# Pixel-Talk/CanonSwap

Hardware: AMD Instinct MI355X
Metric: frames/sec at 512x512 (generator hot path F->W->T->R->W->G) (higher is better)
Workload: dtype f16; 1 GPU; BASELINE configs[2]: 512x512 video, 64 frames batched per launch on each GPU, steady state over 1280 frames (20 launches per GPU) (256x256 crops in, random-init weights of the real architecture); frames_per_launch_per_gpu=64, frames_total=1280, parallelism=frame-shard x1, identities_resident=1, latency_mode=False, accumulate=fp32, debug_decodes=False

## Files before the change

canonswap_amd/csrc/vol32.hip:

```cpp
#include "conv_epilogue.h"

namespace {

constexpr int V_TW = 8;
constexpr int V_NC = V_TW + 2;
constexpr int V_CS = 17 * 16;
constexpr int V_RS = V_NC * V_CS;
constexpr int V_WLO = 27 * 2 * 1024;
constexpr int V_SROWS = 8;
enum { V_EPI_F16 = 0,
       V_EPI_RES = 1,
       V_EPI_STAT = 2 };

template <bool SPLIT, int EPI = 0> struct VRing {
    static constexpr int K = SPLIT ? 2 : 4;
    static constexpr int RING = K + 2;
    static constexpr int QS = ((RING * V_RS + 16 + 255) / 256) * 256;
    static constexpr int IMG = 4 * QS;
    static constexpr int NIMG = SPLIT ? 2 : 1;
    static constexpr int AUX = NIMG * IMG;
    static constexpr int RROWS = K + 1;
    static constexpr int RSLOT = 4 * 4096;
    static constexpr int lds(int epi) { return AUX + (SPLIT ? V_WLO : 0) + (epi == 1 ? RROWS * RSLOT : 0); }
};

struct Vol32Params {
    const half_t* in; const half_t* zero;
    int in_sN, in_sH, in_sW;
    int N, H, W;
    const half_t* wgt;
    const float* bias;
    float sl0, sl1;
    const float* res; int res_sN, res_sH, res_sW;
    void* out0; int o0_sN, o0_sH, o0_sW;
    half_t* out1; int o1_sN, o1_sH, o1_sW;
    const float* s2; const float* t2;
    float* stat_out; int stat_nblk;
    int srows;
    const float* xf_y; int xy_sN, xy_sH, xy_sW;
    const float* xf_res; int xr_sN, xr_sH, xr_sW;
    float* xf_out; int xo_sN, xo_sH, xo_sW;
    const float* xf_stats; const float* xf_gamma; const float* xf_beta; float xf_slope;
    int nstrips, nseg, seg_rows, items;
#ifdef V32_TL
    unsigned long long* tl; long tl_cap;
#endif
};

typedef unsigned int u4v __attribute__((ext_vector_type(4)));

#ifdef V32_TL
#define TLS(i) do { __builtin_amdgcn_sched_barrier(0); const unsigned long long t_ = __builtin_amdgcn_s_memtime(); tl_acc[i] += t_ - tl_last; tl_last = t_; \
                    __builtin_amdgcn_sched_barrier(0); } while (0)
#else
#define TLS(i) do { } while (0)
#endif

template <int N> __device__ __forceinline__ void wait_vm() { asm volatile("s_waitcnt vmcnt(%0)" ::"n"(N) : "memory"); }

template <int EPI, bool SPLIT, int XF>
__global__ void __launch_bounds__(256, 1) vol32_kernel(const Vol32Params p)
{
    static_assert(XF == 0 || (SPLIT && EPI == V_EPI_STAT), "transform staging exists for the split-precision statistics kernel");
    extern __shared__ __attribute__((aligned(16))) unsigned char smem[];
    using R = VRing<SPLIT, EPI>;
    constexpr int K = R::K, RING = R::RING, QS = R::QS, IMG = R::IMG, NIMG = R::NIMG;
    constexpr int VOX = SPLIT ? 64 : 32;
    static_assert(!(SPLIT && EPI == V_EPI_RES), "the residual ring and the W_lo fragments share the LDS region after the images");
    constexpr int ND = XF ? 0 : 3 * NIMG + (EPI == V_EPI_RES ? 4 : 0), NR = 0, NS = EPI == V_EPI_F16 ? 2 : (EPI == V_EPI_RES ? 6 : 4);
    constexpr int NW0 = NR + (K - 2) * (ND + NR + NS), NW = NW0 + NS;
    static_assert(NW <= 63, "vmcnt is a 6-bit counter");
    const int tid = threadIdx.x, lane = tid & 63;
    const int wave = __builtin_amdgcn_readfirstlane(tid >> 6);
    const int l15 = lane & 15, l4 = lane >> 4;
#ifdef V32_TL
    unsigned long long tl_acc[10] = {0, 0, 0, 0, 0, 0, 0, 0, 0, 0}, tl_last = __builtin_amdgcn_s_memtime();
#endif

    for (int i = tid * 16; i < NIMG * IMG; i += 256 * 16) *(u4v*)(smem + i) = (u4v){0u, 0u, 0u, 0u};
    h8_t wr[27][2];
    {
        const half_t* wl = p.wgt + ep_lane_row(1, l15) * 32 + l4 * 8;
#pragma unroll
        for (int t = 0; t < 27; ++t) {
            wr[t][0] = *(const h8_t*)(wl + t * 1024 + ep_frag_row(1, 0) * 32);
            wr[t][1] = *(const h8_t*)(wl + t * 1024 + ep_frag_row(1, 1) * 32);
        }
        if constexpr (SPLIT) {
            for (int f = wave; f < 54; f += 4) {
                const h8_t v = *(const h8_t*)(wl + (27 + (f >> 1)) * 1024 + ep_frag_row(1, f & 1) * 32);
                *(h8_t*)(smem + R::AUX + f * 1024 + lane * 16) = v;
            }
        }
    }
    float bias_v[8], s2_v[8], t2_v[8];
#pragma unroll
    for (int r = 0; r < 8; ++r) {
        bias_v[r] = p.bias ? p.bias[l4 * 8 + r] : 0.f;
        s2_v[r] = p.s2 ? p.s2[l4 * 8 + r] : 1.f;
        t2_v[r] = p.s2 ? p.t2[l4 * 8 + r] : 0.f;
    }
    __syncthreads();

    int s_off[3]; bool s_on[3];
#pragma unroll
    for (int j = 0; j < 3; ++j) {
        const int idx = j * 64 + lane, col = idx / 17, ds = idx % 17;
        s_on[j] = idx < V_NC * 17 && ds != 0;
        s_off[j] = col * p.in_sW + (ds - 1) * VOX + wave * 8;
    }
    const int lanebase = l4 * QS + l15 * 16 + (2 * wave) * V_CS;
    const unsigned lane_el = (unsigned)(l15 * 32 + l4 * 8);
    const unsigned char* wlo = smem + R::AUX + lane * 16;

    const int G = (int)gridDim.x;
    int u = (int)blockIdx.x;
    if ((G & 7) == 0) u = (u & 7) * (G >> 3) + (u >> 3);

    for (int item = u; item < p.items; item += G) {
        int t = item;
        const int strip = t % p.nstrips; t /= p.nstrips;
        const int seg = t % p.nseg;
        const int n = t / p.nseg;
        const int w0 = strip * V_TW;
        const int h0 = seg * p.seg_rows, h1 = (h0 + p.seg_rows < p.H) ? h0 + p.seg_rows : p.H;
        bool c_ok[3];
#pragma unroll
        for (int j = 0; j < 3; ++j) {
            const int col = (j * 64 + lane) / 17;
            c_ok[j] = s_on[j] && (unsigned)(w0 - 1 + col) < (unsigned)p.W;
        }
        const half_t* in_n = p.in + (long)n * p.in_sN + (long)(w0 - 1) * p.in_sW;
        const unsigned nb_o0 = (unsigned)(n * p.o0_sN + (w0 + 2 * wave) * p.o0_sW);
        const unsigned nb_o1 = (unsigned)(n * p.o1_sN + (w0 + 2 * wave) * p.o1_sW);
        const unsigned nb_rs = (unsigned)(n * p.res_sN + (w0 + 2 * wave) * p.res_sW);
        auto stage_piece = [&](int r, int slot, int rslot, int q) {
            if (q < 3 * NIMG) {
                const int im = q / 3, j = q % 3;
                const bool rok = (unsigned)r < (unsigned)p.H && r <= h1;
                const half_t* rp = in_n + (long)r * p.in_sH;
                unsigned char* dst = smem + wave * QS + slot * V_RS;
                if (s_on[j]) {
                    const half_t* src = (rok && c_ok[j]) ? rp + s_off[j] + im * 32 : p.zero;
                    __builtin_amdgcn_global_load_lds((const __attribute__((address_space(1))) void*)src,
                                                     (__attribute__((address_space(3))) void*)(dst + im * IMG + j * 1024), 16, 0, 0);
                }
            } else if constexpr (EPI == V_EPI_RES) {
                const int j = q - 3 * NIMG;
                const int rc = (unsigned)r < (unsigned)p.H ? r : 0;
                const float* rsrc = p.res + (nb_rs + (unsigned)(rc * p.res_sH) + lane_el);
                unsigned char* rdst = smem + R::AUX + rslot * R::RSLOT + wave * 4096;
                __builtin_amdgcn_global_load_lds((const __attribute__((address_space(1))) void*)(rsrc + (j >> 1) * p.res_sW + (j & 1) * 4),
                                                 (__attribute__((address_space(3))) void*)(rdst + j * 1024), 16, 0, 0);
            }
        };
        auto stage_row = [&](int r, int slot, int rslot) {
#pragma unroll
            for (int q = 0; q < ND; ++q) stage_piece(r, slot, rslot, q);
        };
        constexpr bool XRES = XF >= 2 && ((XF - 2) & 1) != 0, XWB = XF >= 2 && ((XF - 2) & 2) != 0;
        float4 xr[XF ? 3 : 1][2], xs[XRES ? 3 : 1][2];
        float xsc[XF >= 2 ? 8 : 1], xsh[XF >= 2 ? 8 : 1];
        const int xq = tid & 3;
        if constexpr (XF >= 2) {
#pragma unroll
            for (int r = 0; r < 8; ++r) {
                const int c = xq * 8 + r;
                const float mean = p.xf_stats[((long)n * 32 + c) * 2], rstd = p.xf_stats[((long)n * 32 + c) * 2 + 1];
                xsc[r] = gn_scale(rstd, p.xf_gamma[c]);
                xsh[r] = gn_shift(mean, xsc[r], p.xf_beta[c]);
            }
        }
        int xoff[XF ? 3 : 1]; bool xcok[XF ? 3 : 1];
        if constexpr (XF != 0) {
#pragma unroll
            for (int it = 0; it < 3; ++it) {
                int idx = it * 256 + tid;
                if (idx >= V_NC * 64) idx -= 128;
                const int col = idx >> 6, d = (idx >> 2) & 15;
                xoff[it] = n * p.xy_sN + (w0 - 1 + col) * p.xy_sW + d * 32 + xq * 8;
                xcok[it] = (unsigned)(w0 - 1 + col) < (unsigned)p.W;
            }
        }
        const unsigned xsafe = (unsigned)(n * p.xy_sN + w0 * p.xy_sW + h0 * p.xy_sH + ((tid >> 2) & 15) * 32 + xq * 8);
        auto xf_load_to = [&](int r, int it, float4 (&dr)[2], float4 (&ds)[2]) {
            if constexpr (XF != 0) {
                const bool okl = xcok[it] && (unsigned)r < (unsigned)p.H && r <= h1;
                const unsigned o = okl ? (unsigned)(xoff[it] + r * p.xy_sH) : xsafe;
                const float* y = p.xf_y + o;
                dr[0] = *(const float4*)y; dr[1] = *(const float4*)(y + 4);
                if constexpr (XRES) {
                    const float* x = p.xf_res + o;
                    ds[0] = *(const float4*)x; ds[1] = *(const float4*)(x + 4);
                }
            }
        };
        auto xf_load = [&](int r, int it) { xf_load_to(r, it, xr[it], xs[XRES ? it : 0]); };
        float xa[8];
        auto xf_write_from = [&](int r, int slot, int it, int part, const float4 (&xr)[2], const float4 (&xs)[2]) {
            if constexpr (XF != 0) {
                int idx = it * 256 + tid;
                if (idx >= V_NC * 64) idx -= 128;
                const bool ok = xcok[it] && (unsigned)r < (unsigned)p.H && r <= h1;
#pragma unroll
                for (int k = 0; k < 8; ++k) {
                    if (part >= 0 && (k >> 2) != part) continue;
                    const float v = ((const float*)&xr[k >> 2])[k & 3];
                    if constexpr (XRES) xa[k] = gn_lrelu(v, xsc[k], xsh[k], ((const float*)&xs[k >> 2])[k & 3], p.xf_slope);
                    else if constexpr (XF >= 2) xa[k] = gn_lrelu(v, xsc[k], xsh[k], 0.f, p.xf_slope);
                    else xa[k] = v;
                    if (!ok) xa[k] = 0.f;
                }
                if (part >= 0 && part != 2) return;
                h8_t hi, lo;
#pragma unroll
                for (int k = 0; k < 8; ++k) { hi[k] = (half_t)xa[k]; lo[k] = (half_t)(xa[k] - (float)hi[k]); }
                unsigned char* dst = smem + xq * QS + (idx >> 6) * V_CS + (((idx >> 2) & 15) + 1) * 16 + slot * V_RS;
                *(h8_t*)dst = hi; *(h8_t*)(dst + IMG) = lo;
                if constexpr (XWB) {
                    float* o = ok ? p.xf_out + (unsigned)(xoff[it] + r * p.xy_sH) : (float*)p.zero;
                    *(float4*)o = make_float4(xa[0], xa[1], xa[2], xa[3]); *(float4*)(o + 4) = make_float4(xa[4], xa[5], xa[6], xa[7]);
                }
            }
        };
        auto xf_write = [&](int r, int slot, int it, int part) { xf_write_from(r, slot, it, part, xr[it], xs[XRES ? it : 0]); };
        if constexpr (XF != 0) {
            float4 pr[3][3][2], ps[XRES ? 3 : 1][3][2];
#pragma unroll
            for (int i = 0; i < 3; ++i)
#pragma unroll
                for (int it = 0; it < 3; ++it) xf_load_to(h0 - 1 + i, it, pr[i][it], ps[XRES ? i : 0][it]);
#pragma unroll
            for (int i = 0; i < 3; ++i)
#pragma unroll
                for (int it = 0; it < 3; ++it) xf_write_from(h0 - 1 + i, i, it, -1, pr[i][it], ps[XRES ? i : 0][it]);
        } else {
#pragma unroll
            for (int i = 0; i <= K; ++i) stage_row(h0 - 1 + i, i, i == 0 ? K : i - 1);
        }
        TLS(0);
        __syncthreads();
        TLS(1);

        float ov[2][8]; h8_t ou[2];
        bool have = false;
        int hprev = 0;
        auto store_piece = [&](int k) {
            constexpr int PC = NS / 2;
            const int c = k / PC, w = k % PC;
            const unsigned o = nb_o0 + (unsigned)(hprev * p.o0_sH + c * p.o0_sW) + lane_el;
            if constexpr (EPI != V_EPI_F16) {
                if (w == 0) *(float4*)((float*)p.out0 + o) = make_float4(ov[c][0], ov[c][1], ov[c][2], ov[c][3]);
                if (w == 1) *(float4*)((float*)p.out0 + o + 4) = make_float4(ov[c][4], ov[c][5], ov[c][6], ov[c][7]);
                if constexpr (EPI == V_EPI_RES) {
                    if (w == 2) *(h8_t*)(p.out1 + (nb_o1 + (unsigned)(hprev * p.o1_sH + c * p.o1_sW) + lane_el)) = ou[c];
                }
            } else {
                h8_t x;
#pragma unroll
                for (int r = 0; r < 8; ++r) x[r] = ep_h(ov[c][r]);
                *(h8_t*)((half_t*)p.out0 + o) = x;
            }
        };
        auto flush = [&]() {
#pragma unroll
            for (int k = 0; k < NS; ++k) store_piece(k);
        };
        float st_s[8], st_q[8];
#pragma unroll
        for (int r = 0; r < 8; ++r) { st_s[r] = 0.f; st_q[r] = 0.f; }

        int s0 = 0, r0 = 0;
        for (int h = h0; h < h1; ++h) {
            int sk = s0 + K + 1; sk -= sk >= RING ? RING : 0;
            int rk = r0 + K; rk -= rk >= R::RROWS ? R::RROWS : 0;
            f4_t rr[2][2];
            if constexpr (EPI == V_EPI_RES) {
#pragma unroll
                for (int c = 0; c < 2; ++c)
#pragma unroll
                    for (int i = 0; i < 2; ++i) rr[c][i] = *(const f4_t*)(wlo + r0 * R::RSLOT + wave * 4096 + (c * 2 + i) * 1024);
            }
            int rb[3];
#pragma unroll
            for (int kh = 0; kh < 3; ++kh) { int sl = s0 + kh; sl -= sl >= RING ? RING : 0; rb[kh] = lanebase + sl * V_RS; }
            f4_t acc[2][2];
#pragma unroll
            for (int c = 0; c < 2; ++c)
#pragma unroll
                for (int ci = 0; ci < 2; ++ci) acc[c][ci] = (f4_t){0.f, 0.f, 0.f, 0.f};
            constexpr int NG = SPLIT ? 27 : 9;
            constexpr int XL0 = 4, XW0 = 17;
            h8_t fa[4], fb[4];
            h8_t wa[SPLIT ? 3 : 1][2], wb[SPLIT ? 3 : 1][2];
            auto rd = [&](h8_t (&f)[4], h8_t (&wl2)[SPLIT ? 3 : 1][2], int G2) {
                const int pass = G2 / 9, g = G2 % 9, kd = g / 3, kh = g % 3;
                const int img = (SPLIT && pass == 2) ? IMG : 0;
#pragma unroll
                for (int i = 0; i < 4; ++i) f[i] = *(const h8_t*)(smem + rb[kh] + img + i * V_CS + kd * 16);
                if constexpr (SPLIT) {
                    if (pass == 1) {
#pragma unroll
                        for (int kw = 0; kw < 3; ++kw)
#pragma unroll
                            for (int ci = 0; ci < 2; ++ci) wl2[kw][ci] = *(const h8_t*)(wlo + ((g * 3 + kw) * 2 + ci) * 1024);
                    }
                }
            };
            rd(fa, wa, 0);
#pragma unroll
            for (int G2 = 0; G2 < NG; ++G2) {
                h8_t (&cur)[4] = (G2 & 1) ? fb : fa;
                h8_t (&wcur)[SPLIT ? 3 : 1][2] = (G2 & 1) ? wb : wa;
                h8_t (&wnxt)[SPLIT ? 3 : 1][2] = (G2 & 1) ? wa : wb;
                if constexpr (XF != 0) { if (G2 >= XW0 && G2 < XW0 + 9) xf_write(h + 2, sk, (G2 - XW0) / 3, (G2 - XW0) % 3); }
                if (G2 + 1 < NG) {
                    h8_t (&nxt)[4] = (G2 & 1) ? fa : fb;
                    rd(nxt, wnxt, G2 + 1);
                }
                const int pass = G2 / 9, g = G2 % 9;
#pragma unroll
                for (int kw = 0; kw < 3; ++kw)
#pragma unroll
                    for (int c = 0; c < 2; ++c)
#pragma unroll
                        for (int ci = 0; ci < 2; ++ci) {
                            const h8_t a = (SPLIT && pass == 1) ? wcur[SPLIT ? kw : 0][ci] : wr[g * 3 + kw][ci];
                            acc[c][ci] = __builtin_amdgcn_mfma_f32_16x16x32_f16(a, cur[kw + c], acc[c][ci], 0, 0, 0);
                        }
                if (G2 + 1 < NG) {
                    const int nrd = 4 + ((SPLIT && (G2 + 1) / 9 == 1) ? 6 : 0);
                    const bool conv_here = XF != 0 && G2 >= XW0 && G2 < XW0 + 9;
#pragma unroll
                    for (int i = 0; i < 11; ++i) {
                        __builtin_amdgcn_sched_group_barrier(0x008, 1, 0);
                        if (i < nrd) __builtin_amdgcn_sched_group_barrier(0x100, 1, 0);
                        if (conv_here) __builtin_amdgcn_sched_group_barrier(0x002, 4, 0);
                    }
                }
                __builtin_amdgcn_sched_barrier(0);
                if constexpr (XF == 0) {
                    constexpr int NM = ND + NS;
#pragma unroll
                    for (int m = G2 * NM / NG; m < (G2 + 1) * NM / NG; ++m) {
                        asm volatile("" ::: "memory");
                        if (m < ND) stage_piece(h + K, sk, rk, m);
                        else if (have) store_piece(m - ND);
                        asm volatile("" ::: "memory");
                    }
                    __builtin_amdgcn_sched_barrier(0);
                } else {
                    if (G2 < NS && have) store_piece(G2);
                    if (G2 >= XL0 && G2 < XL0 + 6 && ((G2 - XL0) & 1) == 0) xf_load(h + 2, (G2 - XL0) >> 1);
                    __builtin_amdgcn_sched_barrier(0);
                }
            }
            TLS(4);
#pragma unroll
            for (int c = 0; c < 2; ++c) {
#pragma unroll
                for (int r = 0; r < 8; ++r) {
                    float v = acc[c][r >> 2][r & 3] + bias_v[r];
                    v = lin_act(v, p.sl0);
                    if constexpr (EPI == V_EPI_RES) v += rr[c][r >> 2][r & 3];
                    ov[c][r] = v;
                    if constexpr (EPI == V_EPI_STAT) { st_s[r] += v; st_q[r] = fmaf(v, v, st_q[r]); }
                    if constexpr (EPI == V_EPI_RES) {
                        const float a = v * s2_v[r] + t2_v[r];
                        ou[c][r] = ep_h(lin_act(a, p.sl1));
                    }
                }
            }
            if constexpr (EPI == V_EPI_STAT) {
                if (((h + 1) % p.srows) == 0 || h + 1 == h1) {
                    const int blk = (h / p.srows) * (p.W / 2) + (w0 / 2 + wave);
                    float pa[8], pb[8];
#pragma unroll
                    for (int r = 0; r < 8; ++r) {
                        float a = st_s[r], b = st_q[r];
                        st_s[r] = 0.f; st_q[r] = 0.f;
#pragma unroll
                        for (int o = 1; o < 16; o <<= 1) { a += __shfl_xor(a, o, 64); b += __shfl_xor(b, o, 64); }
                        pa[r] = a; pb[r] = b;
                    }
                    if (l15 == 0) {
                        float4* dst = (float4*)(p.stat_out + (((long)n * p.stat_nblk + blk) * 32 + l4 * 8) * 2);
#pragma unroll
                        for (int r = 0; r < 4; ++r) dst[r] = make_float4(pa[2 * r], pb[2 * r], pa[2 * r + 1], pb[2 * r + 1]);
                    }
                }
            }
            have = true; hprev = h;
            s0 = s0 + 1 == RING ? 0 : s0 + 1;
            r0 = r0 + 1 == R::RROWS ? 0 : r0 + 1;
            TLS(5);
            if constexpr (XF != 0) asm volatile("s_waitcnt lgkmcnt(0)" ::: "memory");
            else if (h > h0 + K - 2) wait_vm<NW>();
            else wait_vm<NW0>();
            TLS(6);
            __builtin_amdgcn_s_barrier();
            asm volatile("" ::: "memory");
            TLS(7);
#ifdef V32_TL
            tl_acc[9] += 1;
#endif
        }
        if (have) flush();
        __syncthreads();
        TLS(8);
    }
#ifdef V32_TL
    if (p.tl && lane == 0) {
        const long wi = (long)blockIdx.x * 4 + wave;
        if (wi < p.tl_cap) {
            unsigned hwid;
            asm volatile("s_getreg_b32 %0, hwreg(HW_REG_HW_ID)" : "=s"(hwid));
            unsigned long long* o = p.tl + wi * 12;
#pragma unroll
            for (int i = 0; i < 10; ++i) o[i] = tl_acc[i];
            o[10] = hwid; o[11] = __builtin_amdgcn_s_memrealtime();
        }
    }
#endif
}

int g_ncu = 0;
#ifdef V32_TL
unsigned long long* g_v32_tl = nullptr;
long g_v32_cap = 0;
#endif

}

#ifdef V32_TL
extern "C" void cs_debug_set_vol32_tl(void* buf, long cap) { g_v32_tl = (unsigned long long*)buf; g_v32_cap = cap; }
#endif

bool vol32_supported(const ConvParams& p)
{
    if (p.KD != 3 || p.KH != 3 || p.KW != 3 || p.Cout_pad != 32 || p.Cout != 32 || p.D != 16 || p.inD != 16 || (p.W % V_TW) != 0) return false;
    if (p.xf_kind) {
        if (!p.hilo || p.Cin != 96 || !p.stat_out || (p.xf_kind != 1 && p.xf_kind != 2) || !p.xf_y.p || p.xf_y.sD != 32) return false;
        if (p.xf_kind == 2 && (!p.xf_stats || !p.xf_gamma || !p.xf_beta)) return false;
        if (p.xf_res.p && (p.xf_kind != 2 || p.xf_res.sD != 32)) return false;
        if (p.xf_out.p && (p.xf_kind != 2 || p.xf_out.sD != 32)) return false;
    } else if (p.hilo ? (p.Cin != 96 || p.in_sD != 64) : (p.Cin != 32 || p.in_sD != 32)) return false;
    if (p.up_shift || p.cg || p.wslot || p.sk_out || p.ragged || p.pixscale || p.stats || p.pool_hw || p.spmul) return false;
    if (p.act0 > ACT_LRELU || p.act1 > ACT_LRELU) return false;
    if (p.res.p && (!p.res_f32 || p.res.sD != 32)) return false;
    if (p.out0.p && p.out0.sD != 32) return false;
    if (p.out1.p && p.out1.sD != 32) return false;
    if (!p.out0.p) return false;
    if (p.hilo && !p.stat_out) return false;
    if (p.stat_out) return p.out0_f32 && !p.res.p && !p.out1.p;
    if (p.res.p) return p.out0_f32 && p.out1.p && !p.hilo;
    return !p.out0_f32 && !p.out1.p;
}

static int vol32_srows(const ConvParams& p) { return p.v32_srows > 0 ? p.v32_srows : V_SROWS; }
int vol32_stat_nblk(const ConvParams& p) { const int sr = vol32_srows(p); return ((p.H + sr - 1) / sr) * (p.W / 2); }

int launch_vol32(const ConvParams& p, hipStream_t st)
{
    if (!vol32_supported(p)) { cs_set_error("vol32: not a 3x3x3 32 -> 32 convolution on a [N][H][W][16][32] volume this kernel supports"); return -1; }
    if (ep_check_extents(p, "vol32")) return -1;
    const long in_span = (long)(p.N - 1) * p.in_sN + (long)(p.H - 1) * p.in_sH + (long)(p.W - 1) * p.in_sW + 1024;
    if (!p.xf_kind && in_span >= (1L << 31)) { cs_set_error("vol32: the input spans 2^31 elements or more"); return -1; }
    if (!g_ncu) {
        int dev = 0, n = 0;
        if (hipGetDevice(&dev) != hipSuccess || hipDeviceGetAttribute(&n, hipDeviceAttributeMultiprocessorCount, dev) != hipSuccess || n < 1) n = 256;
        g_ncu = n;
    }
    Vol32Params k;
    k.in = p.in; k.zero = p.zero; k.in_sN = (int)p.in_sN; k.in_sH = (int)p.in_sH; k.in_sW = (int)p.in_sW;
    k.N = p.N; k.H = p.H; k.W = p.W;
    k.wgt = p.wgt; k.bias = p.bias;
    k.sl0 = p.act0 == ACT_NONE ? 1.f : (p.act0 == ACT_LRELU ? p.slope0 : 0.f);
    k.sl1 = p.act1 == ACT_NONE ? 1.f : (p.act1 == ACT_LRELU ? p.slope1 : 0.f);
    k.res = (const float*)p.res.p; k.res_sN = (int)p.res.sN; k.res_sH = (int)p.res.sH; k.res_sW = (int)p.res.sW;
    k.out0 = p.out0.p; k.o0_sN = (int)p.out0.sN; k.o0_sH = (int)p.out0.sH; k.o0_sW = (int)p.out0.sW;
    k.out1 = (half_t*)p.out1.p; k.o1_sN = (int)p.out1.sN; k.o1_sH = (int)p.out1.sH; k.o1_sW = (int)p.out1.sW;
    k.s2 = p.s2; k.t2 = p.t2;
    k.stat_out = p.stat_out; k.stat_nblk = vol32_stat_nblk(p); k.srows = vol32_srows(p);
    k.xf_y = (const float*)p.xf_y.p; k.xy_sN = (int)p.xf_y.sN; k.xy_sH = (int)p.xf_y.sH; k.xy_sW = (int)p.xf_y.sW;
    k.xf_res = (const float*)p.xf_res.p; k.xr_sN = (int)p.xf_res.sN; k.xr_sH = (int)p.xf_res.sH; k.xr_sW = (int)p.xf_res.sW;
    k.xf_out = (float*)p.xf_out.p; k.xo_sN = (int)p.xf_out.sN; k.xo_sH = (int)p.xf_out.sH; k.xo_sW = (int)p.xf_out.sW;
    k.xf_stats = p.xf_stats; k.xf_gamma = p.xf_gamma; k.xf_beta = p.xf_beta; k.xf_slope = p.xf_slope;
    if (p.xf_kind) {
        auto same = [&](const TDesc& t) { return !t.p || (t.sN == p.xf_y.sN && t.sH == p.xf_y.sH && t.sW == p.xf_y.sW); };
        if (!same(p.xf_res) || !same(p.xf_out)) { cs_set_error("vol32: the transform-staging volumes must share their strides"); return -1; }
        const long lim = 1L << 31;
        auto span = [&](const TDesc& t) { return (long)(p.N - 1) * t.sN + (long)(p.H - 1) * t.sH + (long)(p.W - 1) * t.sW + 512; };
        if (span(p.xf_y) >= lim || (p.xf_res.p && span(p.xf_res) >= lim) || (p.xf_out.p && span(p.xf_out) >= lim)) {
            cs_set_error("vol32: a transform-staging tensor spans 2^31 elements or more"); return -1;
        }
    }
#ifdef V32_TL
    k.tl = g_v32_tl; k.tl_cap = g_v32_cap;
#endif
    k.nstrips = p.W / V_TW;
    int nseg = 1;
    while ((long)p.N * k.nstrips * nseg < g_ncu && (p.H % (nseg * 2 * k.srows)) == 0) nseg *= 2;
    k.seg_rows = (p.H + nseg - 1) / nseg;
    k.nseg = (p.H + k.seg_rows - 1) / k.seg_rows;
    k.items = p.N * k.nstrips * k.nseg;
    int grid = k.items < g_ncu ? k.items : g_ncu;
    if (grid >= 8) grid &= ~7;
    const bool split = p.hilo != 0;
    const int epi = p.stat_out ? V_EPI_STAT : (p.res.p ? V_EPI_RES : V_EPI_F16);
    auto go = [&](auto kern, size_t lds) -> int {
        if (lds > 64 * 1024) {
            hipError_t e = hipFuncSetAttribute((const void*)kern, hipFuncAttributeMaxDynamicSharedMemorySize, (int)lds);
            if (e != hipSuccess) { cs_set_error("vol32: opting into %zu bytes of LDS failed: %s", lds, hipGetErrorString(e)); return -1; }
        }
        hipLaunchKernelGGL(kern, dim3((unsigned)grid), dim3(256), lds, st, k);
        return 0;
    };
    int r = -1;
    if (split) {
        if (epi != V_EPI_STAT) { cs_set_error("vol32: the split-precision kernel exists with the statistics epilogue only"); return -1; }
        if (p.xf_kind == 2) {
            const int v = (p.xf_res.p ? 1 : 0) | (p.xf_out.p ? 2 : 0);
            if (v == 0) r = go(vol32_kernel<V_EPI_STAT, true, 2>, VRing<true, V_EPI_STAT>::lds(V_EPI_STAT));
            else if (v == 1) r = go(vol32_kernel<V_EPI_STAT, true, 3>, VRing<true, V_EPI_STAT>::lds(V_EPI_STAT));
            else if (v == 2) r = go(vol32_kernel<V_EPI_STAT, true, 4>, VRing<true, V_EPI_STAT>::lds(V_EPI_STAT));
            else r = go(vol32_kernel<V_EPI_STAT, true, 5>, VRing<true, V_EPI_STAT>::lds(V_EPI_STAT));
        }
        else if (p.xf_kind == 1) r = go(vol32_kernel<V_EPI_STAT, true, 1>, VRing<true, V_EPI_STAT>::lds(V_EPI_STAT));
        else r = go(vol32_kernel<V_EPI_STAT, true, 0>, VRing<true, V_EPI_STAT>::lds(V_EPI_STAT));
    } else {
        if (epi == V_EPI_STAT) r = go(vol32_kernel<V_EPI_STAT, false, 0>, VRing<false, V_EPI_STAT>::lds(V_EPI_STAT));
        else if (epi == V_EPI_RES) r = go(vol32_kernel<V_EPI_RES, false, 0>, VRing<false, V_EPI_RES>::lds(V_EPI_RES));
        else r = go(vol32_kernel<V_EPI_F16, false, 0>, VRing<false, V_EPI_F16>::lds(V_EPI_F16));
    }
    if (r) return r;
    hipError_t e = hipGetLastError();
    if (e != hipSuccess) { cs_set_error("vol32 launch: %s", hipGetErrorString(e)); return -1; }
    return 0;
}
```

Baseline: 537.3 frames/s.

## Split vol32 split-precision kernel across eight waves with one output fragment each

For the split-precision (hi/lo) statistics variant, the block grows from 4 to 8 waves. Each wave now owns one 16-channel output fragment instead of two, and the hi and lo image staging is divided between the two wave halves. The transform staging is reworked so each wave handles whole columns: two rounds, the second only for waves 0 and 1, with a specialised step loop for each case. The scheduling-group hints are rescaled to the smaller per-wave MFMA count. The aim is more latency hiding per CU and less register pressure per wave. The cost is duplicated feature-fragment LDS reads across waves, more barrier participants, and imbalance between waves.

```diff
diff --git a/canonswap_amd/csrc/vol32.hip b/canonswap_amd/csrc/vol32.hip
--- a/canonswap_amd/csrc/vol32.hip
+++ b/canonswap_amd/csrc/vol32.hip
@@ -58,47 +58,52 @@
 
 template <int N> __device__ __forceinline__ void wait_vm() { asm volatile("s_waitcnt vmcnt(%0)" ::"n"(N) : "memory"); }
 
+template <bool SPLIT> struct VWaves { static constexpr int NWV = SPLIT ? 8 : 4, NT = NWV * 64, NF = SPLIT ? 1 : 2; };
+
 template <int EPI, bool SPLIT, int XF>
-__global__ void __launch_bounds__(256, 1) vol32_kernel(const Vol32Params p)
+__global__ void __launch_bounds__(VWaves<SPLIT>::NT, 1) vol32_kernel(const Vol32Params p)
 {
     static_assert(XF == 0 || (SPLIT && EPI == V_EPI_STAT), "transform staging exists for the split-precision statistics kernel");
     extern __shared__ __attribute__((aligned(16))) unsigned char smem[];
     using R = VRing<SPLIT, EPI>;
     constexpr int K = R::K, RING = R::RING, QS = R::QS, IMG = R::IMG, NIMG = R::NIMG;
     constexpr int VOX = SPLIT ? 64 : 32;
+    constexpr int NWV = VWaves<SPLIT>::NWV, NT = VWaves<SPLIT>::NT;
+    constexpr int NF = VWaves<SPLIT>::NF, NCH = 4 * NF;
     static_assert(!(SPLIT && EPI == V_EPI_RES), "the residual ring and the W_lo fragments share the LDS region after the images");
-    constexpr int ND = XF ? 0 : 3 * NIMG + (EPI == V_EPI_RES ? 4 : 0), NR = 0, NS = EPI == V_EPI_F16 ? 2 : (EPI == V_EPI_RES ? 6 : 4);
+    constexpr int ND = XF ? 0 : 3 + (EPI == V_EPI_RES ? 4 : 0), NR = 0, NS = EPI == V_EPI_F16 ? 2 : (EPI == V_EPI_RES ? 6 : 2 * NF);
     constexpr int NW0 = NR + (K - 2) * (ND + NR + NS), NW = NW0 + NS;
     static_assert(NW <= 63, "vmcnt is a 6-bit counter");
     const int tid = threadIdx.x, lane = tid & 63;
     const int wave = __builtin_amdgcn_readfirstlane(tid >> 6);
     const int l15 = lane & 15, l4 = lane >> 4;
+    const int cp = SPLIT ? (wave & 3) : wave;
+    const int fw = SPLIT ? (wave >> 2) : 0;
 #ifdef V32_TL
     unsigned long long tl_acc[10] = {0, 0, 0, 0, 0, 0, 0, 0, 0, 0}, tl_last = __builtin_amdgcn_s_memtime();
 #endif
 
-    for (int i = tid * 16; i < NIMG * IMG; i += 256 * 16) *(u4v*)(smem + i) = (u4v){0u, 0u, 0u, 0u};
-    h8_t wr[27][2];
+    for (int i = tid * 16; i < NIMG * IMG; i += NT * 16) *(u4v*)(smem + i) = (u4v){0u, 0u, 0u, 0u};
+    h8_t wr[27][NF];
     {
         const half_t* wl = p.wgt + ep_lane_row(1, l15) * 32 + l4 * 8;
 #pragma unroll
-        for (int t = 0; t < 27; ++t) {
-            wr[t][0] = *(const h8_t*)(wl + t * 1024 + ep_frag_row(1, 0) * 32);
-            wr[t][1] = *(const h8_t*)(wl + t * 1024 + ep_frag_row(1, 1) * 32);
-        }
+        for (int t = 0; t < 27; ++t)
+#pragma unroll
+            for (int ci = 0; ci < NF; ++ci) wr[t][ci] = *(const h8_t*)(wl + t * 1024 + ep_frag_row(1, fw + ci) * 32);
         if constexpr (SPLIT) {
-            for (int f = wave; f < 54; f += 4) {
+            for (int f = wave; f < 54; f += NWV) {
                 const h8_t v = *(const h8_t*)(wl + (27 + (f >> 1)) * 1024 + ep_frag_row(1, f & 1) * 32);
                 *(h8_t*)(smem + R::AUX + f * 1024 + lane * 16) = v;
             }
         }
     }
-    float bias_v[8], s2_v[8], t2_v[8];
-#pragma unroll
-    for (int r = 0; r < 8; ++r) {
-        bias_v[r] = p.bias ? p.bias[l4 * 8 + r] : 0.f;
-        s2_v[r] = p.s2 ? p.s2[l4 * 8 + r] : 1.f;
-        t2_v[r] = p.s2 ? p.t2[l4 * 8 + r] : 0.f;
+    float bias_v[NCH], s2_v[NCH], t2_v[NCH];
+#pragma unroll
+    for (int r = 0; r < NCH; ++r) {
+        bias_v[r] = p.bias ? p.bias[l4 * 8 + fw * 4 + r] : 0.f;
+        s2_v[r] = p.s2 ? p.s2[l4 * 8 + fw * 4 + r] : 1.f;
+        t2_v[r] = p.s2 ? p.t2[l4 * 8 + fw * 4 + r] : 0.f;
     }
     __syncthreads();
 
@@ -107,10 +112,10 @@
     for (int j = 0; j < 3; ++j) {
         const int idx = j * 64 + lane, col = idx / 17, ds = idx % 17;
         s_on[j] = idx < V_NC * 17 && ds != 0;
-        s_off[j] = col * p.in_sW + (ds - 1) * VOX + wave * 8;
-    }
-    const int lanebase = l4 * QS + l15 * 16 + (2 * wave) * V_CS;
-    const unsigned lane_el = (unsigned)(l15 * 32 + l4 * 8);
+        s_off[j] = col * p.in_sW + (ds - 1) * VOX + cp * 8 + fw * 32;
+    }
+    const int lanebase = l4 * QS + l15 * 16 + (2 * cp) * V_CS;
+    const unsigned lane_el = (unsigned)(l15 * 32 + l4 * 8 + fw * 4);
     const unsigned char* wlo = smem + R::AUX + lane * 16;
 
     const int G = (int)gridDim.x;
@@ -131,22 +136,22 @@
             c_ok[j] = s_on[j] && (unsigned)(w0 - 1 + col) < (unsigned)p.W;
         }
         const half_t* in_n = p.in + (long)n * p.in_sN + (long)(w0 - 1) * p.in_sW;
-        const unsigned nb_o0 = (unsigned)(n * p.o0_sN + (w0 + 2 * wave) * p.o0_sW);
-        const unsigned nb_o1 = (unsigned)(n * p.o1_sN + (w0 + 2 * wave) * p.o1_sW);
-        const unsigned nb_rs = (unsigned)(n * p.res_sN + (w0 + 2 * wave) * p.res_sW);
+        const unsigned nb_o0 = (unsigned)(n * p.o0_sN + (w0 + 2 * cp) * p.o0_sW);
+        const unsigned nb_o1 = (unsigned)(n * p.o1_sN + (w0 + 2 * cp) * p.o1_sW);
+        const unsigned nb_rs = (unsigned)(n * p.res_sN + (w0 + 2 * cp) * p.res_sW);
         auto stage_piece = [&](int r, int slot, int rslot, int q) {
-            if (q < 3 * NIMG) {
-                const int im = q / 3, j = q % 3;
+            if (q < 3) {
+                const int j = q;
                 const bool rok = (unsigned)r < (unsigned)p.H && r <= h1;
                 const half_t* rp = in_n + (long)r * p.in_sH;
-                unsigned char* dst = smem + wave * QS + slot * V_RS;
+                unsigned char* dst = smem + cp * QS + fw * IMG + slot * V_RS;
                 if (s_on[j]) {
-                    const half_t* src = (rok && c_ok[j]) ? rp + s_off[j] + im * 32 : p.zero;
+                    const half_t* src = (rok && c_ok[j]) ? rp + s_off[j] : p.zero;
                     __builtin_amdgcn_global_load_lds((const __attribute__((address_space(1))) void*)src,
-                                                     (__attribute__((address_space(3))) void*)(dst + im * IMG + j * 1024), 16, 0, 0);
+                                                     (__attribute__((address_space(3))) void*)(dst + j * 1024), 16, 0, 0);
                 }
             } else if constexpr (EPI == V_EPI_RES) {
-                const int j = q - 3 * NIMG;
+                const int j = q - 3;
                 const int rc = (unsigned)r < (unsigned)p.H ? r : 0;
                 const float* rsrc = p.res + (nb_rs + (unsigned)(rc * p.res_sH) + lane_el);
                 unsigned char* rdst = smem + R::AUX + rslot * R::RSLOT + wave * 4096;
@@ -159,7 +164,10 @@
             for (int q = 0; q < ND; ++q) stage_piece(r, slot, rslot, q);
         };
         constexpr bool XRES = XF >= 2 && ((XF - 2) & 1) != 0, XWB = XF >= 2 && ((XF - 2) & 2) != 0;
-        float4 xr[XF ? 3 : 1][2], xs[XRES ? 3 : 1][2];
+        constexpr int NIT = 2;
+        static_assert(XF == 0 || (NT < V_NC * 64 && NIT * NT >= V_NC * 64 && V_NC * 64 - NT == 2 * 64), "round 1 is waves 0 and 1");
+        const bool two = XF != 0 && wave < 2;
+        float4 xr[XF ? NIT : 1][2], xs[XRES ? NIT : 1][2];
         float xsc[XF >= 2 ? 8 : 1], xsh[XF >= 2 ? 8 : 1];
         const int xq = tid & 3;
         if constexpr (XF >= 2) {
@@ -171,22 +179,21 @@
                 xsh[r] = gn_shift(mean, xsc[r], p.xf_beta[c]);
             }
         }
-        int xoff[XF ? 3 : 1]; bool xcok[XF ? 3 : 1];
+        int xoff[XF ? NIT : 1]; bool xcok[XF ? NIT : 1];
+        const int xl = ((tid >> 2) & 15) * 32 + xq * 8;
         if constexpr (XF != 0) {
 #pragma unroll
-            for (int it = 0; it < 3; ++it) {
-                int idx = it * 256 + tid;
-                if (idx >= V_NC * 64) idx -= 128;
-                const int col = idx >> 6, d = (idx >> 2) & 15;
-                xoff[it] = n * p.xy_sN + (w0 - 1 + col) * p.xy_sW + d * 32 + xq * 8;
-                xcok[it] = (unsigned)(w0 - 1 + col) < (unsigned)p.W;
-            }
-        }
-        const unsigned xsafe = (unsigned)(n * p.xy_sN + w0 * p.xy_sW + h0 * p.xy_sH + ((tid >> 2) & 15) * 32 + xq * 8);
+            for (int it = 0; it < NIT; ++it) {
+                const int col = it * NWV + wave;
+                xoff[it] = n * p.xy_sN + (w0 - 1 + col) * p.xy_sW;
+                xcok[it] = (unsigned)(w0 - 1 + ((it * NT + tid) >> 6)) < (unsigned)p.W;
+            }
+        }
+        const int xsafe = n * p.xy_sN + w0 * p.xy_sW + h0 * p.xy_sH;
         auto xf_load_to = [&](int r, int it, float4 (&dr)[2], float4 (&ds)[2]) {
             if constexpr (XF != 0) {
-                const bool okl = xcok[it] && (unsigned)r < (unsigned)p.H && r <= h1;
-                const unsigned o = okl ? (unsigned)(xoff[it] + r * p.xy_sH) : xsafe;
+                const bool okl = xcok[it] & ((unsigned)r < (unsigned)p.H) & (r <= h1);
+                const unsigned o = (unsigned)((okl ? xoff[it] + r * p.xy_sH : xsafe) + xl);
                 const float* y = p.xf_y + o;
                 dr[0] = *(const float4*)y; dr[1] = *(const float4*)(y + 4);
                 if constexpr (XRES) {
@@ -199,9 +206,7 @@
         float xa[8];
         auto xf_write_from = [&](int r, int slot, int it, int part, const float4 (&xr)[2], const float4 (&xs)[2]) {
             if constexpr (XF != 0) {
-                int idx = it * 256 + tid;
-                if (idx >= V_NC * 64) idx -= 128;
-                const bool ok = xcok[it] && (unsigned)r < (unsigned)p.H && r <= h1;
+                const bool ok = xcok[it] & ((unsigned)r < (unsigned)p.H) & (r <= h1);
 #pragma unroll
                 for (int k = 0; k < 8; ++k) {
                     if (part >= 0 && (k >> 2) != part) continue;
@@ -215,34 +220,38 @@
                 h8_t hi, lo;
 #pragma unroll
                 for (int k = 0; k < 8; ++k) { hi[k] = (half_t)xa[k]; lo[k] = (half_t)(xa[k] - (float)hi[k]); }
-                unsigned char* dst = smem + xq * QS + (idx >> 6) * V_CS + (((idx >> 2) & 15) + 1) * 16 + slot * V_RS;
+                unsigned char* dst = smem + xq * QS + (((tid >> 2) & 15) + 1) * 16 + (it * NWV + wave) * V_CS + slot * V_RS;
                 *(h8_t*)dst = hi; *(h8_t*)(dst + IMG) = lo;
                 if constexpr (XWB) {
-                    float* o = ok ? p.xf_out + (unsigned)(xoff[it] + r * p.xy_sH) : (float*)p.zero;
+                    float* o = ok ? p.xf_out + (unsigned)(xoff[it] + r * p.xy_sH + xl) : (float*)p.zero;
                     *(float4*)o = make_float4(xa[0], xa[1], xa[2], xa[3]); *(float4*)(o + 4) = make_float4(xa[4], xa[5], xa[6], xa[7]);
                 }
             }
         };
         auto xf_write = [&](int r, int slot, int it, int part) { xf_write_from(r, slot, it, part, xr[it], xs[XRES ? it : 0]); };
         if constexpr (XF != 0) {
-            float4 pr[3][3][2], ps[XRES ? 3 : 1][3][2];
-#pragma unroll
-            for (int i = 0; i < 3; ++i)
-#pragma unroll
-                for (int it = 0; it < 3; ++it) xf_load_to(h0 - 1 + i, it, pr[i][it], ps[XRES ? i : 0][it]);
-#pragma unroll
-            for (int i = 0; i < 3; ++i)
-#pragma unroll
-                for (int it = 0; it < 3; ++it) xf_write_from(h0 - 1 + i, i, it, -1, pr[i][it], ps[XRES ? i : 0][it]);
+            float4 pr[3][2], ps[XRES ? 3 : 1][2];
+#pragma unroll
+            for (int i = 0; i < 3; ++i) xf_load_to(h0 - 1 + i, 0, pr[i], ps[XRES ? i : 0]);
+#pragma unroll
+            for (int i = 0; i < 3; ++i) {
+                xf_write_from(h0 - 1 + i, i, 0, -1, pr[i], ps[XRES ? i : 0]);
+                if (two) xf_load_to(h0 - 1 + i, 1, pr[i], ps[XRES ? i : 0]);
+            }
+            if (two) {
+#pragma unroll
+                for (int i = 0; i < 3; ++i) xf_write_from(h0 - 1 + i, i, 1, -1, pr[i], ps[XRES ? i : 0]);
+            }
         } else {
 #pragma unroll
             for (int i = 0; i <= K; ++i) stage_row(h0 - 1 + i, i, i == 0 ? K : i - 1);
         }
         TLS(0);
         __syncthreads();
+        if constexpr (XF != 0) __builtin_amdgcn_s_waitcnt(0x0F70);
         TLS(1);
 
-        float ov[2][8]; h8_t ou[2];
+        float ov[2][NCH]; h8_t ou[2];
         bool have = false;
         int hprev = 0;
         auto store_piece = [&](int k) {
@@ -251,7 +260,9 @@
             const unsigned o = nb_o0 + (unsigned)(hprev * p.o0_sH + c * p.o0_sW) + lane_el;
             if constexpr (EPI != V_EPI_F16) {
                 if (w == 0) *(float4*)((float*)p.out0 + o) = make_float4(ov[c][0], ov[c][1], ov[c][2], ov[c][3]);
-                if (w == 1) *(float4*)((float*)p.out0 + o + 4) = make_float4(ov[c][4], ov[c][5], ov[c][6], ov[c][7]);
+                if constexpr (NF == 2) {
+                    if (w == 1) *(float4*)((float*)p.out0 + o + 4) = make_float4(ov[c][4], ov[c][5], ov[c][6], ov[c][7]);
+                }
                 if constexpr (EPI == V_EPI_RES) {
                     if (w == 2) *(h8_t*)(p.out1 + (nb_o1 + (unsigned)(hprev * p.o1_sH + c * p.o1_sW) + lane_el)) = ou[c];
                 }
@@ -266,12 +277,13 @@
 #pragma unroll
             for (int k = 0; k < NS; ++k) store_piece(k);
         };
-        float st_s[8], st_q[8];
-#pragma unroll
-        for (int r = 0; r < 8; ++r) { st_s[r] = 0.f; st_q[r] = 0.f; }
+        float st_s[NCH], st_q[NCH];
+#pragma unroll
+        for (int r = 0; r < NCH; ++r) { st_s[r] = 0.f; st_q[r] = 0.f; }
 
         int s0 = 0, r0 = 0;
-        for (int h = h0; h < h1; ++h) {
+        auto step = [&](int h, auto two_c) {
+            constexpr int NITV = decltype(two_c)::value ? NIT : 1;
             int sk = s0 + K + 1; sk -= sk >= RING ? RING : 0;
             int rk = r0 + K; rk -= rk >= R::RROWS ? R::RROWS : 0;
             f4_t rr[2][2];
@@ -284,16 +296,16 @@
             int rb[3];
 #pragma unroll
             for (int kh = 0; kh < 3; ++kh) { int sl = s0 + kh; sl -= sl >= RING ? RING : 0; rb[kh] = lanebase + sl * V_RS; }
-            f4_t acc[2][2];
+            f4_t acc[2][NF];
 #pragma unroll
             for (int c = 0; c < 2; ++c)
 #pragma unroll
-                for (int ci = 0; ci < 2; ++ci) acc[c][ci] = (f4_t){0.f, 0.f, 0.f, 0.f};
+                for (int ci = 0; ci < NF; ++ci) acc[c][ci] = (f4_t){0.f, 0.f, 0.f, 0.f};
             constexpr int NG = SPLIT ? 27 : 9;
             constexpr int XL0 = 4, XW0 = 17;
             h8_t fa[4], fb[4];
-            h8_t wa[SPLIT ? 3 : 1][2], wb[SPLIT ? 3 : 1][2];
-            auto rd = [&](h8_t (&f)[4], h8_t (&wl2)[SPLIT ? 3 : 1][2], int G2) {
+            h8_t wa[SPLIT ? 3 : 1][NF], wb[SPLIT ? 3 : 1][NF];
+            auto rd = [&](h8_t (&f)[4], h8_t (&wl2)[SPLIT ? 3 : 1][NF], int G2) {
                 const int pass = G2 / 9, g = G2 % 9, kd = g / 3, kh = g % 3;
                 const int img = (SPLIT && pass == 2) ? IMG : 0;
 #pragma unroll
@@ -303,7 +315,7 @@
 #pragma unroll
                         for (int kw = 0; kw < 3; ++kw)
 #pragma unroll
-                            for (int ci = 0; ci < 2; ++ci) wl2[kw][ci] = *(const h8_t*)(wlo + ((g * 3 + kw) * 2 + ci) * 1024);
+                            for (int ci = 0; ci < NF; ++ci) wl2[kw][ci] = *(const h8_t*)(wlo + ((g * 3 + kw) * 2 + fw + ci) * 1024);
                     }
                 }
             };
@@ -311,9 +323,10 @@
 #pragma unroll
             for (int G2 = 0; G2 < NG; ++G2) {
                 h8_t (&cur)[4] = (G2 & 1) ? fb : fa;
-                h8_t (&wcur)[SPLIT ? 3 : 1][2] = (G2 & 1) ? wb : wa;
-                h8_t (&wnxt)[SPLIT ? 3 : 1][2] = (G2 & 1) ? wa : wb;
-                if constexpr (XF != 0) { if (G2 >= XW0 && G2 < XW0 + 9) xf_write(h + 2, sk, (G2 - XW0) / 3, (G2 - XW0) % 3); }
+                h8_t (&wcur)[SPLIT ? 3 : 1][NF] = (G2 & 1) ? wb : wa;
+                h8_t (&wnxt)[SPLIT ? 3 : 1][NF] = (G2 & 1) ? wa : wb;
+                const bool conv_here = XF != 0 && G2 >= XW0 && G2 < XW0 + 3 * NITV;
+                if constexpr (XF != 0) { if (conv_here) xf_write(h + 2, sk, (G2 - XW0) / 3, (G2 - XW0) % 3); }
                 if (G2 + 1 < NG) {
                     h8_t (&nxt)[4] = (G2 & 1) ? fa : fb;
                     rd(nxt, wnxt, G2 + 1);
@@ -324,18 +337,20 @@
 #pragma unroll
                     for (int c = 0; c < 2; ++c)
 #pragma unroll
-                        for (int ci = 0; ci < 2; ++ci) {
+                        for (int ci = 0; ci < NF; ++ci) {
                             const h8_t a = (SPLIT && pass == 1) ? wcur[SPLIT ? kw : 0][ci] : wr[g * 3 + kw][ci];
                             acc[c][ci] = __builtin_amdgcn_mfma_f32_16x16x32_f16(a, cur[kw + c], acc[c][ci], 0, 0, 0);
                         }
                 if (G2 + 1 < NG) {
-                    const int nrd = 4 + ((SPLIT && (G2 + 1) / 9 == 1) ? 6 : 0);
-                    const bool conv_here = XF != 0 && G2 >= XW0 && G2 < XW0 + 9;
-#pragma unroll
-                    for (int i = 0; i < 11; ++i) {
+                    constexpr int NMF = 6 * NF;
+                    const int nrd = 4 + ((SPLIT && (G2 + 1) / 9 == 1) ? 3 * NF : 0);
+                    const int per = (nrd + NMF - 2) / (NMF - 1);
+#pragma unroll
+                    for (int i = 0; i < NMF - 1; ++i) {
                         __builtin_amdgcn_sched_group_barrier(0x008, 1, 0);
-                        if (i < nrd) __builtin_amdgcn_sched_group_barrier(0x100, 1, 0);
-                        if (conv_here) __builtin_amdgcn_sched_group_barrier(0x002, 4, 0);
+                        if (i * per < nrd) __builtin_amdgcn_sched_group_barrier(0x100, 1, 0);
+                        if (per == 2 && i * per + 1 < nrd) __builtin_amdgcn_sched_group_barrier(0x100, 1, 0);
+                        if (conv_here) __builtin_amdgcn_sched_group_barrier(0x002, 8 / NF, 0);
                     }
                 }
                 __builtin_amdgcn_sched_barrier(0);
@@ -351,7 +366,7 @@
                     __builtin_amdgcn_sched_barrier(0);
                 } else {
                     if (G2 < NS && have) store_piece(G2);
-                    if (G2 >= XL0 && G2 < XL0 + 6 && ((G2 - XL0) & 1) == 0) xf_load(h + 2, (G2 - XL0) >> 1);
+                    if (G2 >= XL0 && G2 < XL0 + 2 * NITV && ((G2 - XL0) & 1) == 0) xf_load(h + 2, (G2 - XL0) >> 1);
                     __builtin_amdgcn_sched_barrier(0);
                 }
             }
@@ -359,7 +374,7 @@
 #pragma unroll
             for (int c = 0; c < 2; ++c) {
 #pragma unroll
-                for (int r = 0; r < 8; ++r) {
+                for (int r = 0; r < NCH; ++r) {
                     float v = acc[c][r >> 2][r & 3] + bias_v[r];
                     v = lin_act(v, p.sl0);
                     if constexpr (EPI == V_EPI_RES) v += rr[c][r >> 2][r & 3];
@@ -373,10 +388,10 @@
             }
             if constexpr (EPI == V_EPI_STAT) {
                 if (((h + 1) % p.srows) == 0 || h + 1 == h1) {
-                    const int blk = (h / p.srows) * (p.W / 2) + (w0 / 2 + wave);
-                    float pa[8], pb[8];
-#pragma unroll
-                    for (int r = 0; r < 8; ++r) {
+                    const int blk = (h / p.srows) * (p.W / 2) + (w0 / 2 + cp);
+                    float pa[NCH], pb[NCH];
+#pragma unroll
+                    for (int r = 0; r < NCH; ++r) {
                         float a = st_s[r], b = st_q[r];
                         st_s[r] = 0.f; st_q[r] = 0.f;
 #pragma unroll
@@ -384,9 +399,9 @@
                         pa[r] = a; pb[r] = b;
                     }
                     if (l15 == 0) {
-                        float4* dst = (float4*)(p.stat_out + (((long)n * p.stat_nblk + blk) * 32 + l4 * 8) * 2);
-#pragma unroll
-                        for (int r = 0; r < 4; ++r) dst[r] = make_float4(pa[2 * r], pb[2 * r], pa[2 * r + 1], pb[2 * r + 1]);
+                        float4* dst = (float4*)(p.stat_out + (unsigned)(((n * p.stat_nblk + blk) * 32 + l4 * 8 + fw * 4) * 2));
+#pragma unroll
+                        for (int r = 0; r < NCH / 2; ++r) dst[r] = make_float4(pa[2 * r], pb[2 * r], pa[2 * r + 1], pb[2 * r + 1]);
                     }
                 }
             }
@@ -404,14 +419,16 @@
 #ifdef V32_TL
             tl_acc[9] += 1;
 #endif
-        }
+        };
+        if (two) { for (int h = h0; h < h1; ++h) step(h, std::true_type{}); }
+        else { for (int h = h0; h < h1; ++h) step(h, std::false_type{}); }
         if (have) flush();
         __syncthreads();
         TLS(8);
     }
 #ifdef V32_TL
     if (p.tl && lane == 0) {
-        const long wi = (long)blockIdx.x * 4 + wave;
+        const long wi = (long)blockIdx.x * NWV + wave;
         if (wi < p.tl_cap) {
             unsigned hwid;
             asm volatile("s_getreg_b32 %0, hwreg(HW_REG_HW_ID)" : "=s"(hwid));
@@ -466,6 +483,7 @@
     if (ep_check_extents(p, "vol32")) return -1;
     const long in_span = (long)(p.N - 1) * p.in_sN + (long)(p.H - 1) * p.in_sH + (long)(p.W - 1) * p.in_sW + 1024;
     if (!p.xf_kind && in_span >= (1L << 31)) { cs_set_error("vol32: the input spans 2^31 elements or more"); return -1; }
+    if (p.stat_out && (long)p.N * vol32_stat_nblk(p) * 64 >= (1L << 31)) { cs_set_error("vol32: the partial statistics span 2^31 elements or more"); return -1; }
     if (!g_ncu) {
         int dev = 0, n = 0;
         if (hipGetDevice(&dev) != hipSuccess || hipDeviceGetAttribute(&n, hipDeviceAttributeMultiprocessorCount, dev) != hipSuccess || n < 1) n = 256;
@@ -513,7 +531,7 @@
             hipError_t e = hipFuncSetAttribute((const void*)kern, hipFuncAttributeMaxDynamicSharedMemorySize, (int)lds);
             if (e != hipSuccess) { cs_set_error("vol32: opting into %zu bytes of LDS failed: %s", lds, hipGetErrorString(e)); return -1; }
         }
-        hipLaunchKernelGGL(kern, dim3((unsigned)grid), dim3(256), lds, st, k);
+        hipLaunchKernelGGL(kern, dim3((unsigned)grid), dim3(split ? VWaves<true>::NT : VWaves<false>::NT), lds, st, k);
         return 0;
     };
     int r = -1;
```

Result: no change. 538.6 frames/s, median of 6 (+0.2%).
